# ChainBreak/denoising_diffusion_deep_fake

Hardware: NVIDIA B200
Metric: train_img_per_s (higher is better)
Workload: dtype bf16

## Files before the change

### denoising_diffusion_deep_fake_b200/csrc/common.cuh

```cuda
#pragma once
#include <cuda_runtime.h>
#include <cuda_bf16.h>
#include <stdint.h>
#include <stdio.h>
#include <string.h>
#include "../../include/d3fk.h"

namespace d3fk {

extern int64_t g_launch_count;
extern char g_last_error[512];
extern int* g_dev_error_flag;

int set_error(int code, const char* fmt, ...);
int check_launch(const char* what);
inline void count_launch(int n = 1) { g_launch_count += n; }

#define D3FK_CHECK_ARG(cond, msg)                                        \
  do {                                                                   \
    if (!(cond)) return d3fk::set_error(D3FK_ERR_ARG, "%s: %s", __func__, msg); \
  } while (0)

static inline int cdiv(long long a, long long b) { return (int)((a + b - 1) / b); }

extern int g_use_pdl;
template <typename... KArgs, typename... Args>
static inline cudaError_t launch_k(void (*kernel)(KArgs...), dim3 grid, dim3 block, size_t smem, cudaStream_t s, dim3 cluster,
                                   Args&&... args) {
  cudaLaunchConfig_t cfg;
  memset(&cfg, 0, sizeof(cfg));
  cfg.gridDim = grid;
  cfg.blockDim = block;
  cfg.dynamicSmemBytes = smem;
  cfg.stream = s;
  cudaLaunchAttribute attr[2];
  int na = 0;
  if (cluster.x * cluster.y * cluster.z > 1) {
    attr[na].id = cudaLaunchAttributeClusterDimension;
    attr[na].val.clusterDim.x = cluster.x;
    attr[na].val.clusterDim.y = cluster.y;
    attr[na].val.clusterDim.z = cluster.z;
    ++na;
  }
  if (g_use_pdl) {
    attr[na].id = cudaLaunchAttributeProgrammaticStreamSerialization;
    attr[na].val.programmaticStreamSerializationAllowed = 1;
    ++na;
  }
  cfg.attrs = attr;
  cfg.numAttrs = na;
  return cudaLaunchKernelEx(&cfg, kernel, static_cast<KArgs>(args)...);
}
#ifdef __CUDACC__
__device__ __forceinline__ void grid_barrier_arrive_wait(unsigned* counter, unsigned expected, int* errflag) {
  asm volatile("red.release.gpu.global.add.u32 [%0], 1;" ::"l"(counter) : "memory");
  const long long t0 = clock64();
  while (true) {
    unsigned v;
    asm volatile("ld.acquire.gpu.global.u32 %0, [%1];" : "=r"(v) : "l"(counter) : "memory");
    if (v >= expected) break;
    if (clock64() - t0 > 4000000000ll) {
      atomicExch(errflag, 2);
      printf("[d3fk] grid barrier timeout: block %d of %d saw %u arrivals (expected %u), counter %p\n", (int)blockIdx.x, (int)gridDim.x, v,
             expected, (void*)counter);
      __trap();
    }
  }
}

__device__ __forceinline__ void pdl_enter() {
  asm volatile("griddepcontrol.wait;" ::: "memory");
  asm volatile("griddepcontrol.launch_dependents;" ::: "memory");
}
#endif

template <typename T> struct Vec;
template <> struct Vec<float> {
  static constexpr int N = 4;
  float v[4];
};
template <> struct Vec<__nv_bfloat16> {
  static constexpr int N = 8;
  __nv_bfloat16 v[8];
};

template <typename T> __device__ __forceinline__ float to_f(T x);
template <> __device__ __forceinline__ float to_f<float>(float x) { return x; }
template <> __device__ __forceinline__ float to_f<__nv_bfloat16>(__nv_bfloat16 x) { return __bfloat162float(x); }
template <typename T> __device__ __forceinline__ T from_f(float x);
template <> __device__ __forceinline__ float from_f<float>(float x) { return x; }
template <> __device__ __forceinline__ __nv_bfloat16 from_f<__nv_bfloat16>(float x) { return __float2bfloat16_rn(x); }

template <typename T> __device__ __forceinline__ void load_vec(const T* p, float* out) {
  constexpr int N = Vec<T>::N;
  uint4 raw = *reinterpret_cast<const uint4*>(p);
  const T* e = reinterpret_cast<const T*>(&raw);
#pragma unroll
  for (int i = 0; i < N; ++i) out[i] = to_f<T>(e[i]);
}
template <typename T> __device__ __forceinline__ uint4 load_raw(const T* p) { return *reinterpret_cast<const uint4*>(p); }
template <typename T> __device__ __forceinline__ void unpack_vec(const uint4& raw, float* out) {
  constexpr int N = Vec<T>::N;
  const T* e = reinterpret_cast<const T*>(&raw);
#pragma unroll
  for (int i = 0; i < N; ++i) out[i] = to_f<T>(e[i]);
}
template <typename T> __device__ __forceinline__ void store_vec(T* p, const float* in) {
  constexpr int N = Vec<T>::N;
  uint4 raw;
  T* e = reinterpret_cast<T*>(&raw);
#pragma unroll
  for (int i = 0; i < N; ++i) e[i] = from_f<T>(in[i]);
  *reinterpret_cast<uint4*>(p) = raw;
}

__device__ __forceinline__ uint4 philox4x32_10(uint4 c, uint2 k) {
  const uint32_t M0 = 0xD2511F53u, M1 = 0xCD9E8D57u, W0 = 0x9E3779B9u, W1 = 0xBB67AE85u;
#pragma unroll
  for (int r = 0; r < 10; ++r) {
    uint32_t hi0 = __umulhi(M0, c.x), lo0 = M0 * c.x;
    uint32_t hi1 = __umulhi(M1, c.z), lo1 = M1 * c.z;
    c = make_uint4(hi1 ^ c.y ^ k.x, lo1, hi0 ^ c.w ^ k.y, lo0);
    k.x += W0;
    k.y += W1;
  }
  return c;
}
__device__ __forceinline__ float u32_to_uniform(uint32_t u) { return ((float)u + 0.5f) * 2.3283064365386963e-10f; }
__device__ __forceinline__ float4 philox_normal4(uint64_t seed, uint64_t idx, uint64_t offset) {
  uint4 c = make_uint4((uint32_t)idx, (uint32_t)(idx >> 32), (uint32_t)offset, (uint32_t)(offset >> 32));
  uint4 r = philox4x32_10(c, make_uint2((uint32_t)seed, (uint32_t)(seed >> 32)));
  float u0 = u32_to_uniform(r.x), u1 = u32_to_uniform(r.y), u2 = u32_to_uniform(r.z), u3 = u32_to_uniform(r.w);
  float ra = sqrtf(-2.f * __logf(u0)), rb = sqrtf(-2.f * __logf(u2));
  float s0, c0, s1, c1;
  __sincosf(6.283185307179586f * u1, &s0, &c0);
  __sincosf(6.283185307179586f * u3, &s1, &c1);
  return make_float4(ra * c0, ra * s0, rb * c1, rb * s1);
}

struct Gather {
  const void* src0; const void* src1;
  int c0, c1, ld0, ld1, up0;
  int B, Hi, Wi, Ho, Wo, kh, kw, stride, pad, mode;
  int ctot;
  int K;
  int M;
  int sshift;
};

__device__ __forceinline__ long long gather_offset(const Gather& g, int n, int h0, int w0, int khi, int kwi, int c,
// ... 28 lines not shown
```

### denoising_diffusion_deep_fake_b200/csrc/conv_tc.cu

```cuda
#include "tc_common.cuh"

namespace d3fk {

template <int BN, int PATH, int FUSE> struct ConvCfg {
  static constexpr int STAGES = BN >= 128 ? ((PATH == 2 && FUSE == 3) ? 6 : 3) : 4;
  static constexpr int B_STAGE_BYTES = BN * 128;
  static constexpr int SMEM = 1024 + STAGES * (A_STAGE_BYTES + B_STAGE_BYTES) + 256 + 10 * BN * 4;
  static constexpr int ACC_COLS = BN < 32 ? 32 : BN;
  static constexpr int TMEM_COLS = 2 * ACC_COLS;
};

struct TileSched {
  int MT, NT, KS, kb_per_split, nkb, total, a_ca;
  int bw, bh, bn, wt, ht;
  int off_w, off_h;
  int a_pitch;
};

__device__ __forceinline__ void decode_tile(const TileSched& ts, int t, int& mt, int& nt, int& ks) {
  if (ts.KS > 1) {
    ks = t % ts.KS;
    const int r = t / ts.KS;
    mt = r % ts.MT;
    nt = r / ts.MT;
  } else {
    ks = 0;
    mt = t % ts.MT;
    nt = t / ts.MT;
  }
}

struct FuseBN {
  const float* gamma; const float* beta;
  float* mean; float* invstd; float* running_mean; float* running_var; long long* nbt;
  float* scale; float* shift;
  bf16* act; const bf16* res;
  unsigned* barrier;
  long long count;
  int ldact, ldr, relu;
  float eps, momentum;
};

template <int BN, int PATH, int FUSE>
__global__ void __launch_bounds__(TC_THREADS, 2) conv_tc_kernel(Gather g, FastDiv dWo, FastDiv dHo, const __grid_constant__ CUtensorMap tmA,
                                                             const __grid_constant__ CUtensorMap tmB, EpiTC e, TileSched ts,
                                                             FuseBN fb, int* errflag) {
  using Cfg = ConvCfg<BN, PATH, FUSE>;
  constexpr int STAGES = Cfg::STAGES;
  constexpr int CW = BN >= 32 ? 32 : 16;
  extern __shared__ uint8_t smem_raw[];
  const uint32_t base = (smem_u32(smem_raw) + 1023u) & ~1023u;
  const uint32_t a_base = base;
  const uint32_t b_base = base + STAGES * A_STAGE_BYTES;
  const uint32_t bar_base = b_base + STAGES * Cfg::B_STAGE_BYTES;
  uint8_t* gen_bar = smem_raw + (base - smem_u32(smem_raw)) + STAGES * (A_STAGE_BYTES + Cfg::B_STAGE_BYTES);
  volatile uint32_t* tmem_ptr_slot = reinterpret_cast<volatile uint32_t*>(gen_bar + 8 * (2 * STAGES + 4));
  float* s_stat = reinterpret_cast<float*>(gen_bar + 256);
  float* s_aff = s_stat + 8 * BN;
  constexpr bool affine = FUSE == 3;
  auto full_bar = [&](int s) { return bar_base + 8u * s; };
  auto empty_bar = [&](int s) { return bar_base + 8u * (STAGES + s); };
  auto acc_full_bar = [&](int b) { return bar_base + 8u * (2 * STAGES + b); };
  auto acc_empty_bar = [&](int b) { return bar_base + 8u * (2 * STAGES + 2 + b); };
  const uint32_t recv_bar = bar_base + 8u * (2 * STAGES + 5);

  const int tid = threadIdx.x, warp = warp_index_uniform(), lane = tid & 31;
  const bool is_epi = warp < 4 || warp >= 6;
  const int q = warp & 3;
  const int half = warp >= 6 ? 1 : 0;
  const int etid = warp < 4 ? tid : 128 + (tid - 192);
  auto stage_affine = [&](int nt, bool live) {
    asm volatile("bar.sync 1, 256;" ::: "memory");
    const int ch = nt * BN + etid;
    if (etid < BN) {
      s_aff[etid] = e.scale ? (live && ch < e.Cout ? __ldg(e.scale + ch) : 0.f) : 1.f;
      s_aff[BN + etid] = live && ch < e.Cout ? __ldg(e.shift + ch) : 0.f;
    }
    asm volatile("bar.sync 1, 256;" ::: "memory");
  };
  const bool clus = ts.KS > 1;
  const bool do_stats = e.stats != nullptr;
  TL_DECL
  TL_BEGIN

  if (tid == 0) {
    for (int s = 0; s < STAGES; ++s) {
      mbar_init(full_bar(s), PATH == 2 ? 1 : 129);
      mbar_init(empty_bar(s), 1);
    }
    for (int b = 0; b < 2; ++b) {
      mbar_init(acc_full_bar(b), 1);
      mbar_init(acc_empty_bar(b), EPI_THREADS);
    }
    mbar_init(recv_bar, 1);
    fence_barrier_init();
  }
  if (is_epi) {
    for (int i = etid; i < 8 * BN; i += EPI_THREADS) s_stat[i] = 0.f;
  }
  if (warp == 5 && elect_one_sync()) {
    tma_prefetch_desc(&tmB);
    if (PATH == 2) tma_prefetch_desc(&tmA);
    int mt0, nt0, ks0;
    decode_tile(ts, blockIdx.x, mt0, nt0, ks0);
    const int kbp = ks0 * ts.kb_per_split;
    for (int i = 0; i < STAGES && kbp + i < ts.nkb; ++i) tma_prefetch_l2_2d(&tmB, (kbp + i) * TC_BK, nt0 * BN);
  }
  if (FUSE == 2 && is_epi && e.bw_x) {
    int mt0, nt0, ks0;
    decode_tile(ts, blockIdx.x, mt0, nt0, ks0);
    const long long mp = (long long)mt0 * TC_BM + q * 32 + lane;
    if (mp < g.M) {
      for (int b = half * 128; b < BN * 2; b += 256) {
        prefetch_l2(reinterpret_cast<const char*>(e.bw_x + mp * e.bw_ldx + nt0 * BN) + b);
        if (e.bw_relu) prefetch_l2(reinterpret_cast<const char*>(e.bw_act + mp * e.bw_ldact + nt0 * BN) + b);
      }
    }
  }
  if (warp == 4) tmem_alloc(smem_u32((const void*)tmem_ptr_slot), Cfg::TMEM_COLS);
  tc_fence_before();
  __syncthreads();
  tc_fence_after();
  const uint32_t tmem_d = *tmem_ptr_slot;
  if (tid == 0) { TL_STAMP(1) }

  auto flush_stats = [&](int nt) {
    asm volatile("bar.sync 1, 256;" ::: "memory");
    const int n0 = nt * BN;
    if (tid < BN && n0 + tid < e.Cout) {
      const float a = (s_stat[tid] + s_stat[2 * BN + tid]) + (s_stat[4 * BN + tid] + s_stat[6 * BN + tid]);
      const float b = (s_stat[BN + tid] + s_stat[3 * BN + tid]) + (s_stat[5 * BN + tid] + s_stat[7 * BN + tid]);
      if (a != 0.f || b != 0.f) {
        atomicAdd(&e.stats[n0 + tid], (double)a);
        atomicAdd(&e.stats[e.Cout + n0 + tid], (FUSE == 2 && e.bw_x) ? bw_second_sum((double)a, (double)b, e, n0 + tid) : (double)b);
      }
    }
    asm volatile("bar.sync 1, 256;" ::: "memory");
    for (int i = etid; i < 8 * BN; i += EPI_THREADS) s_stat[i] = 0.f;
    asm volatile("bar.sync 1, 256;" ::: "memory");
  };

  auto fuse_finalize = [&](int nt, bool publisher) {
    asm volatile("bar.sync 1, 256;" ::: "memory");
    if (tid == 0) grid_barrier_arrive_wait(fb.barrier, gridDim.x, errflag);
    asm volatile("bar.sync 1, 256;" ::: "memory");
    const int ch = nt * BN + tid;
    if (tid < BN && ch < e.Cout) {
      const double n = (double)fb.count;
      const double mean = __ldcg(e.stats + ch) / n;
      double var = __ldcg(e.stats + e.Cout + ch) / n - mean * mean;
      if (var < 0) var = 0;
      const double invstd = rsqrt(var + (double)fb.eps);
      const double gm = (double)__ldg(fb.gamma + ch), bt = (double)__ldg(fb.beta + ch);
      s_stat[tid] = (float)(gm * invstd);
      s_stat[BN + tid] = (float)(bt - mean * gm * invstd);
      if (publisher) {
        fb.mean[ch] = (float)mean;
        fb.invstd[ch] = (float)invstd;
        if (fb.scale) { fb.scale[ch] = s_stat[tid]; fb.shift[ch] = s_stat[BN + tid]; }
        if (fb.running_mean) {
          const double unbiased = n > 1 ? var * n / (n - 1) : var;
          fb.running_mean[ch] = (float)((1.0 - fb.momentum) * fb.running_mean[ch] + fb.momentum * mean);
          fb.running_var[ch] = (float)((1.0 - fb.momentum) * fb.running_var[ch] + fb.momentum * unbiased);
        }
        if (ch == 0 && fb.nbt) *fb.nbt += 1;
      }
    }
    asm volatile("bar.sync 1, 256;" ::: "memory");
  };
  auto fuse_apply = [&](float* f, int ncol, long long m, bool row_ok, int nt, int ct) {
    if (!row_ok) return;
    const int cbase = nt * BN + ct;
    for (int q = 0; q < ncol / 8; ++q) {
      float y[8];
#pragma unroll
      for (int i = 0; i < 8; ++i)
        y[i] = fmaf(__bfloat162float(__float2bfloat16_rn(f[q * 8 + i])), s_stat[ct + q * 8 + i], s_stat[BN + ct + q * 8 + i]);
      if (fb.res) {
        const uint4 rr = __ldg(reinterpret_cast<const uint4*>(fb.res + m * fb.ldr + cbase + q * 8));
        const bf16* rb16 = reinterpret_cast<const bf16*>(&rr);
#pragma unroll
        for (int i = 0; i < 8; ++i) y[i] += __bfloat162float(rb16[i]);
      }
      if (fb.relu) {
#pragma unroll
        for (int i = 0; i < 8; ++i) y[i] = fmaxf(y[i], 0.f);
      }
      uint4 o;
      __nv_bfloat162* o2 = reinterpret_cast<__nv_bfloat162*>(&o);
#pragma unroll
      for (int i = 0; i < 4; ++i) o2[i] = __floats2bfloat162_rn(y[2 * i], y[2 * i + 1]);
      *reinterpret_cast<uint4*>(fb.act + m * fb.ldact + cbase + q * 8) = o;
    }
  };

  if (warp == 5) {
    pdl_enter();
    if (tid == 160) { TL_STAMP(2) }
    if (elect_one_sync()) {
      uint32_t kbg = 0;
      const int sgn = g.mode ? -1 : 1;
      for (int t = blockIdx.x; t < ts.total; t += gridDim.x) {
        int mt, nt, ks;
        decode_tile(ts, t, mt, nt, ks);
        const int kb0 = ks * ts.kb_per_split;
        const int kb1 = min(ts.nkb, kb0 + ts.kb_per_split);
        int w0 = 0, h0 = 0, i0 = 0, tap = 0, c = 0, khi = 0, kwi = 0;
        if (PATH == 2) {
          const int tw = mt % ts.wt;
          const int r2 = mt / ts.wt;
          w0 = tw * ts.bw + ts.off_w;
          h0 = (r2 % ts.ht) * ts.bh + ts.off_h;
          i0 = (r2 / ts.ht) * ts.bn;
          const int k = kb0 * TC_BK;
          tap = k / g.ctot;
          c = k - tap * g.ctot;
          khi = tap / g.kw;
          kwi = tap - khi * g.kw;
        }
        for (int kb = kb0; kb < kb1; ++kb, ++kbg) {
          const int s = kbg % STAGES;
          if (kbg >= STAGES) mbar_wait(empty_bar(s), ((kbg / STAGES) - 1) & 1, errflag);
          mbar_arrive_expect_tx(full_bar(s), Cfg::B_STAGE_BYTES + (PATH == 2 ? A_STAGE_BYTES : 0));
          tma_load_2d(b_base + s * Cfg::B_STAGE_BYTES, &tmB, kb * TC_BK, nt * BN, full_bar(s));
          if (PATH == 2) {
            tma_load_4d(a_base + s * A_STAGE_BYTES, &tmA, c, w0 + sgn * kwi, h0 + sgn * khi, i0, full_bar(s));
            c += TC_BK;
            if (c >= g.ctot) {
              c = 0;
              if (++kwi == g.kw) { kwi = 0; ++khi; }
            }
          }
        }
      }
    }
    __syncwarp();
    if (clus) cluster_sync_relaxed();
  } else if (warp == 4) {
    pdl_enter();
    if (elect_one_sync()) {
      constexpr uint32_t idesc = make_idesc(TC_BM, BN, 0, 0);
      uint32_t kbg = 0, tile_iter = 0;
      for (int t = blockIdx.x; t < ts.total; t += gridDim.x, ++tile_iter) {
        int mt, nt, ks;
        decode_tile(ts, t, mt, nt, ks);
        const int kb0 = ks * ts.kb_per_split;
        const int kb1 = min(ts.nkb, kb0 + ts.kb_per_split);
        const uint32_t abuf = tile_iter & 1;
        if (tile_iter >= 2) {
          mbar_wait(acc_empty_bar(abuf), ((tile_iter >> 1) - 1) & 1, errflag);
          tc_fence_after();
        }
        const uint32_t d_addr = tmem_d + abuf * Cfg::ACC_COLS;
        for (int kb = kb0; kb < kb1; ++kb, ++kbg) {
          const int s = kbg % STAGES;
          mbar_wait(full_bar(s), (kbg / STAGES) & 1, errflag);
          if (kbg == 0) { TL_STAMP(3) }
          tc_fence_after();
          const uint32_t a_addr = a_base + s * A_STAGE_BYTES;
          const uint32_t b_addr = b_base + s * Cfg::B_STAGE_BYTES;
#pragma unroll
          for (int kk = 0; kk < TC_BK / 16; ++kk) {
// ... 37 lines not shown
        const int kb1 = min(ts.nkb, kb0 + ts.kb_per_split);

        if (PATH != 2 && warp < 4 && live) {
          int rh[8], rw[8];
          int rn[8];
          const bf16* rp[8];
#pragma unroll
          for (int i = 0; i < 8; ++i) {
            const int m = m0 + rb + 16 * i;
            int n = 0, h0 = -(1 << 28), w0 = 0;
            if (m < g.M) {
              const uint32_t qq = fdiv((uint32_t)m, dWo);
              const int wo = m - (int)qq * g.Wo;
              n = (int)fdiv(qq, dHo);
              const int ho = (int)qq - n * g.Ho;
              if (g.mode == 0) { h0 = ho * g.stride - g.pad; w0 = wo * g.stride - g.pad; }
              else { h0 = ho + g.pad; w0 = wo + g.pad; }
            }
            rh[i] = h0; rw[i] = w0;
            if (PATH == 0) rp[i] = (const bf16*)g.src0 + ((long long)(n * g.Hi + h0) * g.Wi + w0) * g.ld0;
            else rn[i] = n;
          }
          int k = kb0 * TC_BK + j * 8;
          int tap = k / g.ctot;
          int c = k - tap * g.ctot;
          int khi = tap / g.kw, kwi = tap - khi * g.kw;

          for (int kb = kb0; kb < kb1; ++kb, ++kbg) {
            const int s = kbg % STAGES;
            if (kbg >= STAGES) mbar_wait(empty_bar(s), ((kbg / STAGES) - 1) & 1, errflag);
            const bool k_ok = k < g.K;
            const uint32_t a_dst = a_base + s * A_STAGE_BYTES + rb * 128 + sw;
            const int dkh = sgn * khi, dkw = sgn * kwi;
            if (PATH == 0) {
              const long long koff = (long long)(dkh * g.Wi + dkw) * g.ld0 + c;
#pragma unroll
              for (int i = 0; i < 8; ++i) {
                const bool ok = k_ok && (unsigned)(rh[i] + dkh) < (unsigned)g.Hi && (unsigned)(rw[i] + dkw) < (unsigned)g.Wi;
                const void* src = ok ? (const void*)(rp[i] + koff) : g.src0;
                if (ts.a_ca) cp_async_16_ca(a_dst + i * (16 * 128), src, ok ? 16u : 0u);
                else cp_async_16(a_dst + i * (16 * 128), src, ok ? 16u : 0u);
              }
            } else {
              const bool second = c >= g.c0;
              const bf16* sb = second ? (const bf16*)g.src1 + (c - g.c0) : (const bf16*)g.src0 + c;
              const int ld = second ? g.ld1 : g.ld0;
              const int up = second ? 0 : g.up0;
              const int hs = g.Hi >> up, wsz = g.Wi >> up;
#pragma unroll
              for (int i = 0; i < 8; ++i) {
                const int th = rh[i] + dkh, tw = rw[i] + dkw;
                const int hi = th >> sshift, wi = tw >> sshift;
                const bool ok = k_ok && (((uint32_t)(th | tw)) & (0x80000000u | smask)) == 0 && hi < g.Hi && wi < g.Wi;
                const long long pix = (long long)((rn[i] * hs + (hi >> up)) * wsz + (wi >> up));
                const void* src = ok ? (const void*)(sb + pix * ld) : g.src0;
                if (ts.a_ca) cp_async_16_ca(a_dst + i * (16 * 128), src, ok ? 16u : 0u);
                else cp_async_16(a_dst + i * (16 * 128), src, ok ? 16u : 0u);
              }
            }
            cp_async_mbar_arrive(full_bar(s));
            mbar_arrive(full_bar(s));
            k += TC_BK;
            c += TC_BK;
            while (c >= g.ctot) {
              c -= g.ctot;
              if (++kwi == g.kw) { kwi = 0; ++khi; }
            }
          }
        }

        const uint32_t abuf = tile_iter & 1;
        if (live) {
          mbar_wait(acc_full_bar(abuf), (tile_iter >> 1) & 1, errflag);
          if (tid == 0) { TL_STAMP(5) }
          tc_fence_after();
        }
        const int m = m0 + row;
        const bool row_ok = live && m < g.M;
        if (!clus) {
          if (affine && (cur_aff_nt != nt || !live)) {
            stage_affine(nt, live);
            cur_aff_nt = live ? nt : -1;
          }
          if (live && do_stats && cur_nt != nt) {
            if (cur_nt >= 0) flush_stats(cur_nt);
            cur_nt = nt;
          }
          int on = 0, oh = 0, ow = 0;
          if (e.out_nchw && row_ok) {
            const uint32_t qq = fdiv((uint32_t)m, dWo);
            ow = m - (int)qq * e.Wo;
            on = (int)fdiv(qq, dHo);
            oh = (int)qq - on * e.Ho;
          }
#pragma unroll 1
          for (int cc = half * CW; cc < BN; cc += 2 * CW) {
            uint32_t raw[CW];
            const uint32_t taddr = tmem_d + ((uint32_t)(q * 32) << 16) + abuf * Cfg::ACC_COLS + (uint32_t)cc;
            const bool tstats = do_stats && !(FUSE == 2 && e.bw_x);
            if (tstats) tmem_col_stats<CW>(taddr, live ? g.M - (m0 + q * 32) : 0, s_stat + q * 2 * BN + cc, s_stat + q * 2 * BN + BN + cc, lane);
            if (CW == 32) tmem_ld32(taddr, raw); else tmem_ld16(taddr, raw);
            tmem_ld_wait();
            float f[CW];
#pragma unroll
            for (int i = 0; i < CW; ++i) f[i] = __uint_as_float(raw[i]);
            epilogue_chunk<CW, FUSE == 2>(f, e, (long long)m, row_ok, n0 + cc, on, oh, ow, do_stats && !tstats, s_stat + q * 2 * BN + cc,
                                          s_stat + q * 2 * BN + BN + cc, lane, affine ? s_aff + cc : nullptr, BN);
            if (tid == 0 && cc == 0) { TL_STAMP(8) }
          }
          if (tid == 0) { TL_STAMP(9) }
          if (FUSE == 1 && live) {
            flush_stats(nt);
            cur_nt = -1;
            fuse_finalize(nt, mt == 0);
#pragma unroll 1
            for (int cc = half * CW; cc < BN; cc += 2 * CW) {
              uint32_t raw[CW];
              const uint32_t taddr = tmem_d + ((uint32_t)(q * 32) << 16) + abuf * Cfg::ACC_COLS + (uint32_t)cc;
              if (CW == 32) tmem_ld32(taddr, raw); else tmem_ld16(taddr, raw);
              tmem_ld_wait();
              float f[CW];
#pragma unroll
              for (int i = 0; i < CW; ++i) f[i] = __uint_as_float(raw[i]);
              fuse_apply(f, CW, (long long)m, row_ok, nt, cc);
            }
          }
          if (live) {
            tc_fence_before();
            mbar_arrive(acc_empty_bar(abuf));
          }
        } else {
          const int KS = ts.KS, SL = BN / KS, sl4 = SL >> 2;
          const uint32_t rank = cluster_ctarank();
          const uint32_t recv = a_base;
          if (live) {
            if (etid == 0) mbar_arrive_expect_tx(recv_bar, (uint32_t)(TC_BM * BN * 4));
            tc_fence_before();
            cluster_sync_relaxed();
            tc_fence_after();
            if (tid == 0) { TL_STAMP(11) }
          }
#pragma unroll 1
          for (int cc = half * CW; cc < BN; cc += 2 * CW) {
            uint32_t raw[CW];
            const uint32_t taddr = tmem_d + ((uint32_t)(q * 32) << 16) + (uint32_t)cc;
            if (CW == 32) tmem_ld32(taddr, raw); else tmem_ld16(taddr, raw);
            tmem_ld_wait();
#pragma unroll
            for (int q4 = 0; q4 < CW / 4; ++q4) {
              const int col = cc + 4 * q4;
              const int owner = col / SL, within = col - owner * SL;
              const uint32_t la = recv + (uint32_t)((((int)rank * sl4 + (within >> 2)) * 128 + row) * 16);
              const uint32_t ra = mapa_shared(la, (uint32_t)owner);
              if (live) st_async_f4(ra, raw[4 * q4], raw[4 * q4 + 1], raw[4 * q4 + 2], raw[4 * q4 + 3], mapa_shared(recv_bar, (uint32_t)owner));
            }
          }
          if (live) {
            if (tid == 0) { TL_STAMP(12) }
            mbar_wait(recv_bar, 0, errflag);
            if (tid == 0) { TL_STAMP(13) }
          }
          if (affine) stage_affine(nt, live);
          const int cslice = (int)rank * SL;
#pragma unroll 1
          for (int ch = half * 16; ch < SL; ch += 32) {
            float f[16];
#pragma unroll
            for (int c4 = 0; c4 < 4; ++c4) {
              float4 a = make_float4(0.f, 0.f, 0.f, 0.f);
              for (int r = 0; r < KS; ++r) {
                const float4 v = ld_shared_f4(recv + (uint32_t)(((r * sl4 + (ch >> 2) + c4) * 128 + row) * 16));
                a.x += v.x; a.y += v.y; a.z += v.z; a.w += v.w;
              }
              f[4 * c4] = a.x; f[4 * c4 + 1] = a.y; f[4 * c4 + 2] = a.z; f[4 * c4 + 3] = a.w;
            }
            const int ct = cslice + ch;
            const bool tstats = do_stats && !(FUSE == 2 && e.bw_x);
            if (tstats) {
              const uint32_t taddr = tmem_d + ((uint32_t)(q * 32) << 16) + (uint32_t)ct;
              if (live) tmem_st16(taddr, f);
              __syncwarp();
              tmem_col_stats<16>(taddr, live ? g.M - (m0 + q * 32) : 0, s_stat + q * 2 * BN + ct, s_stat + q * 2 * BN + BN + ct, lane);
            }
            epilogue_chunk<16, FUSE == 2>(f, e, (long long)m, row_ok, nt * BN + ct, 0, 0, 0, do_stats && !tstats, s_stat + q * 2 * BN + ct,
                                          s_stat + q * 2 * BN + BN + ct, lane, affine ? s_aff + ct : nullptr, BN);
          }
          if (tid == 0) { TL_STAMP(14) }
          if (live && do_stats) flush_stats(nt);
          if (tid == 0) { TL_STAMP(15) }
          if (FUSE == 1 && live) {
            fuse_finalize(nt, mt == 0 && rank == 0);
#pragma unroll 1
            for (int ch = half * 16; ch < SL; ch += 32) {
              float f[16];
#pragma unroll
              for (int c4 = 0; c4 < 4; ++c4) {
                float4 a = make_float4(0.f, 0.f, 0.f, 0.f);
                for (int r = 0; r < KS; ++r) {
                  const float4 v = ld_shared_f4(recv + (uint32_t)(((r * sl4 + (ch >> 2) + c4) * 128 + row) * 16));
                  a.x += v.x; a.y += v.y; a.z += v.z; a.w += v.w;
                }
                f[4 * c4] = a.x; f[4 * c4 + 1] = a.y; f[4 * c4 + 2] = a.z; f[4 * c4 + 3] = a.w;
              }
              fuse_apply(f, 16, (long long)m, row_ok, nt, cslice + ch);
            }
          }
        }
        if (!live || clus) break;
      }
      if (tid == 0) { TL_STAMP(10) }
      if (live && !clus && do_stats && cur_nt >= 0) flush_stats(cur_nt);
    }
  }

  if (tid == 0) { TL_STAMP(6) }
  tc_fence_before();
  __syncthreads();
  if (warp == 4) tmem_dealloc(tmem_d, Cfg::TMEM_COLS);
  if (tid == 128) { TL_STAMP(7) }
}

int g_num_sms = 148;
int g_verbose = 0;
int g_max_cluster = 8;
static int g_tile_loop = 1;
static int g_a_ca = 0;
static int g_occ_cap = 0;
static int g_use_tma_a = 1;
static int g_split_tiles = 74;
static int g_split_cta_cap = 100;

struct FuseReq { const d3fk_bn_params* bn; unsigned* barrier; bool taken; };
static thread_local FuseReq* t_fuse = nullptr;
static int g_fuse_bn = 1;

template <int BN, int PATH>
static int launch_conv_tc_bn(const Gather& g, const d3fk_conv_params* p, cudaStream_t s, const TileSched& box) {
  EpiTC e{(bf16*)p->out, p->out_nchw, p->scale, p->shift, (const bf16*)p->res, p->stats, p->ldo, p->ldr, p->relu, p->Cout, p->Ho, p->Wo,
           (const bf16*)p->bw_x, (const bf16*)p->bw_act, p->bw_mean, p->bw_invstd, p->bw_ldx, p->bw_ldact, p->bw_relu};
  TileSched ts = box;
  ts.MT = cdiv(g.M, TC_BM);
  ts.NT = cdiv(p->Cout, BN);
  ts.nkb = cdiv(g.K, TC_BK);
  ts.KS = 1;
  const int tiles = ts.MT * ts.NT;
  ts.a_ca = g_a_ca && p->kh > 1;
  if (BN == 128 && !p->out_nchw && p->Cout % BN == 0 && tiles <= g_split_tiles && ts.nkb >= 8 && g_max_cluster > 1) {
    int ks = 1;
    while (ks * 2 <= g_max_cluster && ks * 2 <= 8 && tiles * ks * 2 <= g_split_cta_cap * g_num_sms / 100 && ts.nkb / (ks * 2) >= 4) ks *= 2;
    while (ks > 1 && tiles * ks > cluster_capacity(ks, 2)) ks >>= 1;
    ts.KS = ks;
  }
  ts.kb_per_split = cdiv(ts.nkb, ts.KS);
  if (ts.KS > 1 && (ts.KS - 1) * ts.kb_per_split >= ts.nkb) {
    ts.KS = 1;
    ts.kb_per_split = ts.nkb;
  }
  ts.total = tiles * ts.KS;
  const bool eval_affine = !p->bw_x && (p->scale || p->shift);
  const int smem_bytes = eval_affine ? ConvCfg<BN, PATH, 3>::SMEM : ConvCfg<BN, PATH, 0>::SMEM;
  int occ = (227 * 1024) / (smem_bytes + 1024);
  if (occ * ConvCfg<BN, PATH, 0>::TMEM_COLS > 512) occ = 512 / ConvCfg<BN, PATH, 0>::TMEM_COLS;
  if (g_occ_cap > 0 && occ > g_occ_cap) occ = g_occ_cap;
  int grid = ts.total < g_num_sms * occ ? ts.total : g_num_sms * occ;
  if (!g_tile_loop || ts.KS > 1) grid = ts.total;

  alignas(64) CUtensorMap tmA, tmB;
  memset(&tmA, 0, sizeof(tmA));
  {
    uint64_t dims[2] = {(uint64_t)g.K, (uint64_t)p->Cout};
    uint64_t strides[1] = {(uint64_t)g.K * 2};
    uint32_t bx[2] = {TC_BK, (uint32_t)BN};
    int rc = get_tensor_map(&tmB, p->w, 2, dims, strides, bx, 128);
    if (rc) return rc;
  }
  if (PATH == 2) {
    uint64_t dims[4] = {(uint64_t)g.c0, (uint64_t)g.Wi, (uint64_t)g.Hi, (uint64_t)g.B};
    const uint64_t pitch = (uint64_t)(ts.a_pitch ? ts.a_pitch : g.Wi);
    uint64_t strides[3] = {(uint64_t)g.ld0 * 2, pitch * g.ld0 * 2, (uint64_t)g.Hi * pitch * g.ld0 * 2};
    uint32_t bx[4] = {TC_BK, (uint32_t)ts.bw, (uint32_t)ts.bh, (uint32_t)ts.bn};
    int rc = get_tensor_map(&tmA, p->src0, 4, dims, strides, bx, 128);
    if (rc) return rc;
  }
  FuseBN fb;
  memset(&fb, 0, sizeof(fb));
  bool fuse = false;
  if (BN == 128 && t_fuse && g_fuse_bn && p->stats && !p->scale && !p->shift && !p->res && !p->relu && !p->out_nchw && p->mode == 0 &&
      p->Cout % BN == 0 && ts.total <= cluster_capacity_safe(ts.KS)) {
// ... 183 lines not shown
```

### denoising_diffusion_deep_fake_b200/csrc/tc_common.cuh

```cuda
#pragma once
#include <stdlib.h>
#include <string.h>
#include "common.cuh"
#include "tma.cuh"

namespace d3fk {

typedef __nv_bfloat16 bf16;

#ifdef D3FK_TIMELINE
#define TL_SLOTS 16
#define TL_MAX 512
__device__ __forceinline__ unsigned long long tl_now() { unsigned long long t; asm volatile("mov.u64 %0, %%globaltimer;" : "=l"(t)); return t; }
#define TL_DECL unsigned long long* tl_buf = reinterpret_cast<unsigned long long*>(errflag + 16); __shared__ unsigned tl_idx;
#define TL_BEGIN if (blockIdx.x == 0 && threadIdx.x == 0) { tl_idx = atomicAdd(reinterpret_cast<unsigned*>(errflag + 4), 1u) % TL_MAX; tl_buf[tl_idx * TL_SLOTS + 0] = tl_now(); }
#define TL_STAMP(slot) if (blockIdx.x == 0) { tl_buf[tl_idx * TL_SLOTS + (slot)] = tl_now(); }
#else
#define TL_DECL
#define TL_BEGIN
#define TL_STAMP(slot)
#endif

__device__ __forceinline__ uint32_t smem_u32(const void* p) { return (uint32_t)__cvta_generic_to_shared(p); }

__device__ __forceinline__ bool elect_one_sync() {
  uint32_t pred;
  asm volatile("{\n\t.reg .pred p;\n\telect.sync _|p, 0xffffffff;\n\tselp.u32 %0, 1, 0, p;\n\t}" : "=r"(pred));
  return pred != 0;
}
__device__ __forceinline__ int warp_index_uniform() { return __shfl_sync(0xffffffffu, (int)(threadIdx.x >> 5), 0); }

__device__ __forceinline__ void mbar_init(uint32_t bar, uint32_t count) {
  asm volatile("mbarrier.init.shared::cta.b64 [%0], %1;" ::"r"(bar), "r"(count) : "memory");
}
__device__ __forceinline__ void mbar_arrive(uint32_t bar) {
  asm volatile("mbarrier.arrive.shared::cta.b64 _, [%0];" ::"r"(bar) : "memory");
}
__device__ __forceinline__ void cp_async_mbar_arrive(uint32_t bar) {
  asm volatile("cp.async.mbarrier.arrive.shared::cta.b64 [%0];" ::"r"(bar) : "memory");
}
__device__ __forceinline__ uint32_t mbar_try_wait(uint32_t bar, uint32_t parity) {
  uint32_t ok;
  asm volatile(
      "{\n\t.reg .pred p;\n\t"
      "mbarrier.try_wait.parity.shared::cta.b64 p, [%1], %2;\n\t"
      "selp.u32 %0, 1, 0, p;\n\t}"
      : "=r"(ok)
      : "r"(bar), "r"(parity)
      : "memory");
  return ok;
}
static __device__ __noinline__ void mbar_timeout(int* errflag, uint32_t bar, uint32_t parity) {
  atomicExch(errflag, 1);
  printf("[d3fk] mbarrier watchdog: block %d thread %d waited > 2 s on barrier 0x%x parity %u\n", (int)blockIdx.x,
         (int)threadIdx.x, bar, parity);
  __trap();
}
__device__ __forceinline__ void mbar_wait(uint32_t bar, uint32_t parity, int* errflag) {
  if (mbar_try_wait(bar, parity)) return;
  unsigned long long t0;
  asm volatile("mov.u64 %0, %%globaltimer;" : "=l"(t0));
  for (uint32_t it = 1;; ++it) {
    if (mbar_try_wait(bar, parity)) return;
    if ((it & 1023u) == 0) {
      unsigned long long t;
      asm volatile("mov.u64 %0, %%globaltimer;" : "=l"(t));
      if (t - t0 > 2000000000ull) mbar_timeout(errflag, bar, parity);
    }
  }
}
__device__ __forceinline__ void cp_async_16(uint32_t dst, const void* src, uint32_t bytes) {
  asm volatile("cp.async.cg.shared.global [%0], [%1], 16, %2;" ::"r"(dst), "l"(src), "r"(bytes) : "memory");
}
__device__ __forceinline__ void cp_async_16_ca(uint32_t dst, const void* src, uint32_t bytes) {
  asm volatile("cp.async.ca.shared.global [%0], [%1], 16, %2;" ::"r"(dst), "l"(src), "r"(bytes) : "memory");
}
__device__ __forceinline__ void fence_proxy_async() { asm volatile("fence.proxy.async.shared::cta;" ::: "memory"); }
__device__ __forceinline__ void fence_barrier_init() { asm volatile("fence.mbarrier_init.release.cluster;" ::: "memory"); }
__device__ __forceinline__ void tc_fence_before() { asm volatile("tcgen05.fence::before_thread_sync;" ::: "memory"); }
__device__ __forceinline__ void tc_fence_after() { asm volatile("tcgen05.fence::after_thread_sync;" ::: "memory"); }

__device__ __forceinline__ void tmem_alloc(uint32_t smem_dst, uint32_t ncols) {
  asm volatile("tcgen05.alloc.cta_group::1.sync.aligned.shared::cta.b32 [%0], %1;" ::"r"(smem_dst), "r"(ncols) : "memory");
  asm volatile("tcgen05.relinquish_alloc_permit.cta_group::1.sync.aligned;" ::: "memory");
}
__device__ __forceinline__ void tmem_dealloc(uint32_t taddr, uint32_t ncols) {
  asm volatile("tcgen05.dealloc.cta_group::1.sync.aligned.b32 %0, %1;" ::"r"(taddr), "r"(ncols) : "memory");
}
__device__ __forceinline__ void umma_f16(uint32_t d_tmem, uint64_t adesc, uint64_t bdesc, uint32_t idesc, uint32_t accumulate) {
  asm volatile(
      "{\n\t.reg .pred p;\n\t"
      "setp.ne.b32 p, %4, 0;\n\t"
      "tcgen05.mma.cta_group::1.kind::f16 [%0], %1, %2, %3, p;\n\t}"
      ::"r"(d_tmem), "l"(adesc), "l"(bdesc), "r"(idesc), "r"(accumulate)
      : "memory");
}
__device__ __forceinline__ void umma_f16_lohi(uint32_t d_tmem, uint32_t alo, uint32_t ahi, uint32_t blo, uint32_t bhi, uint32_t idesc,
                                              uint32_t accumulate) {
  asm volatile(
      "{\n\t.reg .pred p;\n\t.reg .b64 da, db;\n\t"
      "mov.b64 da, {%1, %2};\n\t"
      "mov.b64 db, {%3, %4};\n\t"
      "setp.ne.b32 p, %6, 0;\n\t"
      "tcgen05.mma.cta_group::1.kind::f16 [%0], da, db, %5, p;\n\t}"
      ::"r"(d_tmem), "r"(alo), "r"(ahi), "r"(blo), "r"(bhi), "r"(idesc), "r"(accumulate)
      : "memory");
}
__device__ __forceinline__ void umma_commit(uint32_t bar) {
  asm volatile("tcgen05.commit.cta_group::1.mbarrier::arrive::one.shared::cluster.b64 [%0];" ::"r"(bar) : "memory");
}
__device__ __forceinline__ void tmem_ld32(uint32_t taddr, uint32_t* v) {
  asm volatile(
      "tcgen05.ld.sync.aligned.32x32b.x32.b32 "
      "{%0, %1, %2, %3, %4, %5, %6, %7, %8, %9, %10, %11, %12, %13, %14, %15, "
      "%16, %17, %18, %19, %20, %21, %22, %23, %24, %25, %26, %27, %28, %29, %30, %31}, [%32];"
      : "=r"(v[0]), "=r"(v[1]), "=r"(v[2]), "=r"(v[3]), "=r"(v[4]), "=r"(v[5]), "=r"(v[6]), "=r"(v[7]), "=r"(v[8]),
        "=r"(v[9]), "=r"(v[10]), "=r"(v[11]), "=r"(v[12]), "=r"(v[13]), "=r"(v[14]), "=r"(v[15]), "=r"(v[16]),
        "=r"(v[17]), "=r"(v[18]), "=r"(v[19]), "=r"(v[20]), "=r"(v[21]), "=r"(v[22]), "=r"(v[23]), "=r"(v[24]),
        "=r"(v[25]), "=r"(v[26]), "=r"(v[27]), "=r"(v[28]), "=r"(v[29]), "=r"(v[30]), "=r"(v[31])
      : "r"(taddr)
      : "memory");
}
__device__ __forceinline__ void tmem_ld16(uint32_t taddr, uint32_t* v) {
  asm volatile(
      "tcgen05.ld.sync.aligned.32x32b.x16.b32 "
      "{%0, %1, %2, %3, %4, %5, %6, %7, %8, %9, %10, %11, %12, %13, %14, %15}, [%16];"
      : "=r"(v[0]), "=r"(v[1]), "=r"(v[2]), "=r"(v[3]), "=r"(v[4]), "=r"(v[5]), "=r"(v[6]), "=r"(v[7]), "=r"(v[8]),
        "=r"(v[9]), "=r"(v[10]), "=r"(v[11]), "=r"(v[12]), "=r"(v[13]), "=r"(v[14]), "=r"(v[15])
      : "r"(taddr)
      : "memory");
}
__device__ __forceinline__ void tmem_ld_wait() { asm volatile("tcgen05.wait::ld.sync.aligned;" ::: "memory"); }

__device__ __forceinline__ uint32_t cluster_ctarank() {
  uint32_t r;
  asm volatile("mov.u32 %0, %%cluster_ctarank;" : "=r"(r));
  return r;
}
__device__ __forceinline__ void cluster_sync_all() {
  asm volatile("barrier.cluster.arrive.release.aligned;\n\tbarrier.cluster.wait.acquire.aligned;" ::: "memory");
}
__device__ __forceinline__ void cluster_sync_relaxed() {
  asm volatile("barrier.cluster.arrive.relaxed.aligned;\n\tbarrier.cluster.wait.aligned;" ::: "memory");
}
__device__ __forceinline__ void st_async_f4(uint32_t remote_addr, uint32_t a, uint32_t b, uint32_t c, uint32_t d, uint32_t remote_mbar) {
  asm volatile("st.async.weak.shared::cluster.mbarrier::complete_tx::bytes.v4.b32 [%0], {%1, %2, %3, %4}, [%5];"
               ::"r"(remote_addr), "r"(a), "r"(b), "r"(c), "r"(d), "r"(remote_mbar) : "memory");
}
__device__ __forceinline__ uint32_t mapa_shared(uint32_t addr, uint32_t rank) {
  uint32_t r;
  asm volatile("mapa.shared::cluster.u32 %0, %1, %2;" : "=r"(r) : "r"(addr), "r"(rank));
  return r;
}
__device__ __forceinline__ void st_cluster_f4(uint32_t addr, uint32_t a, uint32_t b, uint32_t c, uint32_t d) {
  asm volatile("st.shared::cluster.v4.b32 [%0], {%1, %2, %3, %4};" ::"r"(addr), "r"(a), "r"(b), "r"(c), "r"(d) : "memory");
}
__device__ __forceinline__ float4 ld_shared_f4(uint32_t addr) {
  float4 v;
  asm volatile("ld.shared.v4.f32 {%0, %1, %2, %3}, [%4];" : "=f"(v.x), "=f"(v.y), "=f"(v.z), "=f"(v.w) : "r"(addr) : "memory");
  return v;
}

__device__ __forceinline__ uint64_t make_smem_desc(uint32_t saddr, uint32_t lbo_bytes, uint32_t sbo_bytes) {
  uint64_t d = 0;
  d |= (uint64_t)((saddr & 0x3FFFFu) >> 4);
  d |= (uint64_t)((lbo_bytes >> 4) & 0x3FFFu) << 16;
  d |= (uint64_t)((sbo_bytes >> 4) & 0x3FFFu) << 32;
  d |= (uint64_t)1 << 46;
  d |= (uint64_t)2 << 61;
  return d;
}
__host__ __device__ constexpr uint32_t make_idesc(int M, int N, int a_mn_major, int b_mn_major) {
  return (1u << 4) | (1u << 7) | (1u << 10) | ((uint32_t)a_mn_major << 15) | ((uint32_t)b_mn_major << 16) |
         ((uint32_t)(N >> 3) << 17) | ((uint32_t)(M >> 4) << 24);
}

__device__ __forceinline__ float warp_colsum32(float* v, int lane) {
#pragma unroll
  for (int ofs = 16, n = 32; ofs >= 1; ofs >>= 1, n >>= 1) {
    const bool up = (lane & ofs) != 0;
#pragma unroll
    for (int i = 0; i < n / 2; ++i) {
      float send = up ? v[i] : v[i + n / 2];
      float keep = up ? v[i + n / 2] : v[i];
      v[i] = keep + __shfl_xor_sync(0xffffffffu, send, ofs);
    }
  }
  return v[0];
}
__device__ __forceinline__ float warp_colsum16(float* v, int lane) {
#pragma unroll
  for (int i = 0; i < 16; ++i) v[i] += __shfl_xor_sync(0xffffffffu, v[i], 16);
#pragma unroll
  for (int ofs = 8, n = 16; ofs >= 1; ofs >>= 1, n >>= 1) {
    const bool up = (lane & ofs) != 0;
#pragma unroll
    for (int i = 0; i < n / 2; ++i) {
      float send = up ? v[i] : v[i + n / 2];
      float keep = up ? v[i + n / 2] : v[i];
      v[i] = keep + __shfl_xor_sync(0xffffffffu, send, ofs);
    }
  }
  return v[0];
}

template <int NREP> __device__ __forceinline__ void tmem_ld_16x256b(uint32_t taddr, uint32_t* v);
template <> __device__ __forceinline__ void tmem_ld_16x256b<4>(uint32_t taddr, uint32_t* v) {
  asm volatile(
      "tcgen05.ld.sync.aligned.16x256b.x4.b32 "
      "{%0, %1, %2, %3, %4, %5, %6, %7, %8, %9, %10, %11, %12, %13, %14, %15}, [%16];"
      : "=r"(v[0]), "=r"(v[1]), "=r"(v[2]), "=r"(v[3]), "=r"(v[4]), "=r"(v[5]), "=r"(v[6]), "=r"(v[7]), "=r"(v[8]),
        "=r"(v[9]), "=r"(v[10]), "=r"(v[11]), "=r"(v[12]), "=r"(v[13]), "=r"(v[14]), "=r"(v[15])
      : "r"(taddr)
      : "memory");
}
template <> __device__ __forceinline__ void tmem_ld_16x256b<2>(uint32_t taddr, uint32_t* v) {
  asm volatile("tcgen05.ld.sync.aligned.16x256b.x2.b32 {%0, %1, %2, %3, %4, %5, %6, %7}, [%8];"
               : "=r"(v[0]), "=r"(v[1]), "=r"(v[2]), "=r"(v[3]), "=r"(v[4]), "=r"(v[5]), "=r"(v[6]), "=r"(v[7])
               : "r"(taddr)
               : "memory");
}
__device__ __forceinline__ void tmem_st16(uint32_t taddr, const float* f) {
  asm volatile(
      "tcgen05.st.sync.aligned.32x32b.x16.b32 [%0], {%1, %2, %3, %4, %5, %6, %7, %8, %9, %10, %11, %12, %13, %14, %15, %16};"
      ::"r"(taddr), "f"(f[0]), "f"(f[1]), "f"(f[2]), "f"(f[3]), "f"(f[4]), "f"(f[5]), "f"(f[6]), "f"(f[7]), "f"(f[8]), "f"(f[9]),
        "f"(f[10]), "f"(f[11]), "f"(f[12]), "f"(f[13]), "f"(f[14]), "f"(f[15])
      : "memory");
  asm volatile("tcgen05.wait::st.sync.aligned;" ::: "memory");
}
template <int CW>
__device__ __forceinline__ void tmem_col_stats(uint32_t taddr, int row_limit, float* sstat_sum, float* sstat_sq, int lane) {
  constexpr int J = CW / 8;
  uint32_t a[4 * J], b[4 * J];
  tmem_ld_16x256b<J>(taddr, a);
  tmem_ld_16x256b<J>(taddr + (16u << 16), b);
  tmem_ld_wait();
  const int r0 = lane >> 2;
  const bool v0 = r0 < row_limit, v1 = r0 + 8 < row_limit, v2 = r0 + 16 < row_limit, v3 = r0 + 24 < row_limit;
// ... 183 lines not shown
```

Measured before the change: 73970.

## Split fused-BN grid barrier into arrive/wait and overlap with epilogue work

The fused conv+BN epilogue (FUSE==1) previously did a combined arrive-and-wait grid barrier before any output processing. The barrier is now split: each block arrives right after accumulating its channel stats. While other blocks arrive, it prefetches residual tiles into shared memory via cp.async, loads gamma/beta and running stats, and runs a pre-barrier output pass. It then waits and applies normalization with the staged residual and vectorized scale/shift reads. This hides barrier latency and global residual-load latency, at the cost of a second TMEM read pass and reuse of A-stage shared memory as residual staging. The cluster split-K path also seems to drop its old cross-rank reduction sum in favor of reading TMEM directly.

```diff
diff --git a/denoising_diffusion_deep_fake_b200/csrc/common.cuh b/denoising_diffusion_deep_fake_b200/csrc/common.cuh
--- a/denoising_diffusion_deep_fake_b200/csrc/common.cuh
+++ b/denoising_diffusion_deep_fake_b200/csrc/common.cuh
@@ -52,8 +52,10 @@
   return cudaLaunchKernelEx(&cfg, kernel, static_cast<KArgs>(args)...);
 }
 #ifdef __CUDACC__
-__device__ __forceinline__ void grid_barrier_arrive_wait(unsigned* counter, unsigned expected, int* errflag) {
+__device__ __forceinline__ void grid_barrier_arrive(unsigned* counter) {
   asm volatile("red.release.gpu.global.add.u32 [%0], 1;" ::"l"(counter) : "memory");
+}
+__device__ __forceinline__ void grid_barrier_wait(unsigned* counter, unsigned expected, int* errflag) {
   const long long t0 = clock64();
   while (true) {
     unsigned v;
@@ -66,6 +68,10 @@
       __trap();
     }
   }
+}
+__device__ __forceinline__ void grid_barrier_arrive_wait(unsigned* counter, unsigned expected, int* errflag) {
+  grid_barrier_arrive(counter);
+  grid_barrier_wait(counter, expected, errflag);
 }
 
 __device__ __forceinline__ void pdl_enter() {
diff --git a/denoising_diffusion_deep_fake_b200/csrc/conv_tc.cu b/denoising_diffusion_deep_fake_b200/csrc/conv_tc.cu
--- a/denoising_diffusion_deep_fake_b200/csrc/conv_tc.cu
+++ b/denoising_diffusion_deep_fake_b200/csrc/conv_tc.cu
@@ -47,6 +47,8 @@
                                                              FuseBN fb, int* errflag) {
   using Cfg = ConvCfg<BN, PATH, FUSE>;
   constexpr int STAGES = Cfg::STAGES;
+  static_assert(FUSE != 1 || (STAGES * A_STAGE_BYTES >= TC_BM * BN * 2 &&
+                              STAGES * (A_STAGE_BYTES + Cfg::B_STAGE_BYTES) >= TC_BM * BN * 5), "FUSE 1 residual staging");
   constexpr int CW = BN >= 32 ? 32 : 16;
   extern __shared__ uint8_t smem_raw[];
   const uint32_t base = (smem_u32(smem_raw) + 1023u) & ~1023u;
@@ -67,6 +69,7 @@
   const int tid = threadIdx.x, warp = warp_index_uniform(), lane = tid & 31;
   const bool is_epi = warp < 4 || warp >= 6;
   const int q = warp & 3;
+  const int erow = q * 32 + lane;
   const int half = warp >= 6 ? 1 : 0;
   const int etid = warp < 4 ? tid : 128 + (tid - 192);
   auto stage_affine = [&](int nt, bool live) {
@@ -140,44 +143,85 @@
     asm volatile("bar.sync 1, 256;" ::: "memory");
   };
 
-  auto fuse_finalize = [&](int nt, bool publisher) {
+  auto fuse_arrive = [&](int nt, bool live) {
     asm volatile("bar.sync 1, 256;" ::: "memory");
-    if (tid == 0) grid_barrier_arrive_wait(fb.barrier, gridDim.x, errflag);
+    const int n0 = nt * BN;
+    if (live && tid < BN && n0 + tid < e.Cout) {
+      const float a = (s_stat[tid] + s_stat[2 * BN + tid]) + (s_stat[4 * BN + tid] + s_stat[6 * BN + tid]);
+      const float b = (s_stat[BN + tid] + s_stat[3 * BN + tid]) + (s_stat[5 * BN + tid] + s_stat[7 * BN + tid]);
+      if (a != 0.f || b != 0.f) {
+        atomicAdd(&e.stats[n0 + tid], (double)a);
+        atomicAdd(&e.stats[e.Cout + n0 + tid], (double)b);
+      }
+    }
     asm volatile("bar.sync 1, 256;" ::: "memory");
-    const int ch = nt * BN + tid;
-    if (tid < BN && ch < e.Cout) {
+    if (tid == 0) { TL_STAMP(16) }
+    if (live && tid == 0) grid_barrier_arrive(fb.barrier);
+    if (tid == 0) { TL_STAMP(17) }
+  };
+  const int fch = tid;
+  float f_gamma = 0.f, f_beta = 0.f, f_rmean = 0.f, f_rvar = 0.f;
+  double f_mean = 0.0, f_var = 0.0, f_invstd = 0.0;
+  auto fuse_load_params = [&](int nt, bool publisher) {
+    const int ch = nt * BN + fch;
+    if (fch < BN && ch < e.Cout) {
+      f_gamma = __ldg(fb.gamma + ch);
+      f_beta = __ldg(fb.beta + ch);
+      if (publisher && fb.running_mean) { f_rmean = fb.running_mean[ch]; f_rvar = fb.running_var[ch]; }
+    }
+  };
+  auto fuse_wait = [&](int nt) {
+    if (tid == 0) grid_barrier_wait(fb.barrier, gridDim.x, errflag);
+    if (tid == 0) { TL_STAMP(18) }
+    asm volatile("bar.sync 1, 256;" ::: "memory");
+    const int ch = nt * BN + fch;
+    if (fch < BN && ch < e.Cout) {
       const double n = (double)fb.count;
-      const double mean = __ldcg(e.stats + ch) / n;
-      double var = __ldcg(e.stats + e.Cout + ch) / n - mean * mean;
-      if (var < 0) var = 0;
-      const double invstd = rsqrt(var + (double)fb.eps);
-      const double gm = (double)__ldg(fb.gamma + ch), bt = (double)__ldg(fb.beta + ch);
-      s_stat[tid] = (float)(gm * invstd);
-      s_stat[BN + tid] = (float)(bt - mean * gm * invstd);
-      if (publisher) {
-        fb.mean[ch] = (float)mean;
-        fb.invstd[ch] = (float)invstd;
-        if (fb.scale) { fb.scale[ch] = s_stat[tid]; fb.shift[ch] = s_stat[BN + tid]; }
-        if (fb.running_mean) {
-          const double unbiased = n > 1 ? var * n / (n - 1) : var;
-          fb.running_mean[ch] = (float)((1.0 - fb.momentum) * fb.running_mean[ch] + fb.momentum * mean);
-          fb.running_var[ch] = (float)((1.0 - fb.momentum) * fb.running_var[ch] + fb.momentum * unbiased);
-        }
-        if (ch == 0 && fb.nbt) *fb.nbt += 1;
-      }
+      f_mean = __ldcg(e.stats + ch) / n;
+      f_var = __ldcg(e.stats + e.Cout + ch) / n - f_mean * f_mean;
+      if (f_var < 0) f_var = 0;
+      f_invstd = rsqrt(f_var + (double)fb.eps);
+      const double gm = (double)f_gamma, bt = (double)f_beta;
+      s_stat[fch] = (float)(gm * f_invstd);
+      s_stat[BN + fch] = (float)(bt - f_mean * gm * f_invstd);
     }
     asm volatile("bar.sync 1, 256;" ::: "memory");
+    if (tid == 0) { TL_STAMP(19) }
   };
-  auto fuse_apply = [&](float* f, int ncol, long long m, bool row_ok, int nt, int ct) {
+  auto fuse_publish = [&](int nt) {
+    const int ch = nt * BN + fch;
+    if (fch < BN && ch < e.Cout) {
+      fb.mean[ch] = (float)f_mean;
+      fb.invstd[ch] = (float)f_invstd;
+      if (fb.scale) { fb.scale[ch] = s_stat[fch]; fb.shift[ch] = s_stat[BN + fch]; }
+      if (fb.running_mean) {
+        const double n = (double)fb.count;
+        const double unbiased = n > 1 ? f_var * n / (n - 1) : f_var;
+        fb.running_mean[ch] = (float)((1.0 - fb.momentum) * f_rmean + fb.momentum * f_mean);
+        fb.running_var[ch] = (float)((1.0 - fb.momentum) * f_rvar + fb.momentum * unbiased);
+      }
+      if (ch == 0 && fb.nbt) *fb.nbt += 1;
+    }
+  };
+  auto fuse_fetch_res = [&](uint32_t res_s, long long m, bool row_ok, int cbase, int cj, int ncol) {
+    if (!fb.res || !row_ok) return;
+    for (int q8 = 0; q8 < ncol / 8; ++q8)
+      cp_async_16(res_s + (uint32_t)(((cj + q8) * TC_BM + erow) * 16), fb.res + m * fb.ldr + cbase + q8 * 8, 16u);
+  };
+  auto fuse_apply = [&](float* f, int ncol, long long m, bool row_ok, int nt, int ct, uint32_t res_s, int cj) {
     if (!row_ok) return;
     const int cbase = nt * BN + ct;
     for (int q = 0; q < ncol / 8; ++q) {
-      float y[8];
+      float y[8], sc[8], sh[8];
+      *reinterpret_cast<float4*>(sc) = *reinterpret_cast<const float4*>(s_stat + ct + q * 8);
+      *reinterpret_cast<float4*>(sc + 4) = *reinterpret_cast<const float4*>(s_stat + ct + q * 8 + 4);
+      *reinterpret_cast<float4*>(sh) = *reinterpret_cast<const float4*>(s_stat + BN + ct + q * 8);
+      *reinterpret_cast<float4*>(sh + 4) = *reinterpret_cast<const float4*>(s_stat + BN + ct + q * 8 + 4);
 #pragma unroll
       for (int i = 0; i < 8; ++i)
-        y[i] = fmaf(__bfloat162float(__float2bfloat16_rn(f[q * 8 + i])), s_stat[ct + q * 8 + i], s_stat[BN + ct + q * 8 + i]);
+        y[i] = fmaf(__bfloat162float(__float2bfloat16_rn(f[q * 8 + i])), sc[i], sh[i]);
       if (fb.res) {
-        const uint4 rr = __ldg(reinterpret_cast<const uint4*>(fb.res + m * fb.ldr + cbase + q * 8));
+        const uint4 rr = ld_shared_u4(res_s + (uint32_t)(((cj + q) * TC_BM + erow) * 16));
         const bf16* rb16 = reinterpret_cast<const bf16*>(&rr);
 #pragma unroll
         for (int i = 0; i < 8; ++i) y[i] += __bfloat162float(rb16[i]);
@@ -381,7 +425,7 @@
             stage_affine(nt, live);
             cur_aff_nt = live ? nt : -1;
           }
-          if (live && do_stats && cur_nt != nt) {
+          if (FUSE != 1 && live && do_stats && cur_nt != nt) {
             if (cur_nt >= 0) flush_stats(cur_nt);
             cur_nt = nt;
           }
@@ -392,37 +436,58 @@
             on = (int)fdiv(qq, dHo);
             oh = (int)qq - on * e.Ho;
           }
+          if (FUSE == 1) {
+            const uint32_t tbase = tmem_d + ((uint32_t)(q * 32) << 16) + abuf * Cfg::ACC_COLS;
 #pragma unroll 1
-          for (int cc = half * CW; cc < BN; cc += 2 * CW) {
-            uint32_t raw[CW];
-            const uint32_t taddr = tmem_d + ((uint32_t)(q * 32) << 16) + abuf * Cfg::ACC_COLS + (uint32_t)cc;
-            const bool tstats = do_stats && !(FUSE == 2 && e.bw_x);
-            if (tstats) tmem_col_stats<CW>(taddr, live ? g.M - (m0 + q * 32) : 0, s_stat + q * 2 * BN + cc, s_stat + q * 2 * BN + BN + cc, lane);
-            if (CW == 32) tmem_ld32(taddr, raw); else tmem_ld16(taddr, raw);
-            tmem_ld_wait();
-            float f[CW];
-#pragma unroll
-            for (int i = 0; i < CW; ++i) f[i] = __uint_as_float(raw[i]);
-            epilogue_chunk<CW, FUSE == 2>(f, e, (long long)m, row_ok, n0 + cc, on, oh, ow, do_stats && !tstats, s_stat + q * 2 * BN + cc,
-                                          s_stat + q * 2 * BN + BN + cc, lane, affine ? s_aff + cc : nullptr, BN);
-            if (tid == 0 && cc == 0) { TL_STAMP(8) }
-          }
-          if (tid == 0) { TL_STAMP(9) }
-          if (FUSE == 1 && live) {
-            flush_stats(nt);
-            cur_nt = -1;
-            fuse_finalize(nt, mt == 0);
+            for (int cc = half * CW; cc < BN; cc += 2 * CW)
+              tmem_col_stats<CW>(tbase + (uint32_t)cc, live ? g.M - (m0 + q * 32) : 0,
+                                 s_stat + q * 2 * BN + cc, s_stat + q * 2 * BN + BN + cc, lane);
+            if (tid == 0) { TL_STAMP(9) }
+            fuse_arrive(nt, live);
+            if (live) fuse_load_params(nt, mt == 0);
+#pragma unroll 1
+            for (int cc = half * CW; cc < BN; cc += 2 * CW) {
+              fuse_fetch_res(a_base, (long long)m, row_ok, n0 + cc, cc / 8, CW);
+              uint32_t raw[CW];
+              if (CW == 32) tmem_ld32(tbase + (uint32_t)cc, raw); else tmem_ld16(tbase + (uint32_t)cc, raw);
+              tmem_ld_wait();
+              float f[CW];
+#pragma unroll
+              for (int i = 0; i < CW; ++i) f[i] = __uint_as_float(raw[i]);
+              epilogue_chunk<CW, false>(f, e, (long long)m, row_ok, n0 + cc, 0, 0, 0, false, nullptr, nullptr, lane);
+            }
+            if (tid == 0) { TL_STAMP(20) }
+            if (live) fuse_wait(nt);
+            cp_async_wait_all();
+#pragma unroll 1
+            for (int cc = half * CW; cc < BN; cc += 2 * CW) {
+              uint32_t raw[CW];
+              if (CW == 32) tmem_ld32(tbase + (uint32_t)cc, raw); else tmem_ld16(tbase + (uint32_t)cc, raw);
+              tmem_ld_wait();
+              float f[CW];
+#pragma unroll
+              for (int i = 0; i < CW; ++i) f[i] = __uint_as_float(raw[i]);
+              fuse_apply(f, CW, (long long)m, row_ok, nt, cc, a_base, cc / 8);
+            }
+            if (tid == 0) { TL_STAMP(21) }
+            if (live && mt == 0) fuse_publish(nt);
+          } else {
 #pragma unroll 1
             for (int cc = half * CW; cc < BN; cc += 2 * CW) {
               uint32_t raw[CW];
               const uint32_t taddr = tmem_d + ((uint32_t)(q * 32) << 16) + abuf * Cfg::ACC_COLS + (uint32_t)cc;
+              const bool tstats = do_stats && !(FUSE == 2 && e.bw_x);
+              if (tstats) tmem_col_stats<CW>(taddr, live ? g.M - (m0 + q * 32) : 0, s_stat + q * 2 * BN + cc, s_stat + q * 2 * BN + BN + cc, lane);
               if (CW == 32) tmem_ld32(taddr, raw); else tmem_ld16(taddr, raw);
               tmem_ld_wait();
               float f[CW];
 #pragma unroll
               for (int i = 0; i < CW; ++i) f[i] = __uint_as_float(raw[i]);
-              fuse_apply(f, CW, (long long)m, row_ok, nt, cc);
-            }
+              epilogue_chunk<CW, FUSE == 2>(f, e, (long long)m, row_ok, n0 + cc, on, oh, ow, do_stats && !tstats, s_stat + q * 2 * BN + cc,
+                                            s_stat + q * 2 * BN + BN + cc, lane, affine ? s_aff + cc : nullptr, BN);
+              if (tid == 0 && cc == 0) { TL_STAMP(8) }
+            }
+            if (tid == 0) { TL_STAMP(9) }
           }
           if (live) {
             tc_fence_before();
@@ -481,28 +546,48 @@
               __syncwarp();
               tmem_col_stats<16>(taddr, live ? g.M - (m0 + q * 32) : 0, s_stat + q * 2 * BN + ct, s_stat + q * 2 * BN + BN + ct, lane);
             }
-            epilogue_chunk<16, FUSE == 2>(f, e, (long long)m, row_ok, nt * BN + ct, 0, 0, 0, do_stats && !tstats, s_stat + q * 2 * BN + ct,
-                                          s_stat + q * 2 * BN + BN + ct, lane, affine ? s_aff + ct : nullptr, BN);
+            if (FUSE != 1)
+              epilogue_chunk<16, FUSE == 2>(f, e, (long long)m, row_ok, nt * BN + ct, 0, 0, 0, do_stats && !tstats, s_stat + q * 2 * BN + ct,
+                                            s_stat + q * 2 * BN + BN + ct, lane, affine ? s_aff + ct : nullptr, BN);
           }
           if (tid == 0) { TL_STAMP(14) }
-          if (live && do_stats) flush_stats(nt);
-          if (tid == 0) { TL_STAMP(15) }
-          if (FUSE == 1 && live) {
-            fuse_finalize(nt, mt == 0 && rank == 0);
+          if (FUSE == 1) {
+            const bool publisher = mt == 0 && rank == 0;
+            const uint32_t tbase = tmem_d + ((uint32_t)(q * 32) << 16);
+            const uint32_t res_s = a_base + TC_BM * BN * 4;
+            fuse_arrive(nt, live);
+            if (live) fuse_load_params(nt, publisher);
 #pragma unroll 1
             for (int ch = half * 16; ch < SL; ch += 32) {
+              const int ct = cslice + ch;
+              fuse_fetch_res(res_s, (long long)m, row_ok, nt * BN + ct, ch / 8, 16);
+              uint32_t raw[16];
+              tmem_ld16(tbase + (uint32_t)ct, raw);
+              tmem_ld_wait();
               float f[16];
 #pragma unroll
-              for (int c4 = 0; c4 < 4; ++c4) {
-                float4 a = make_float4(0.f, 0.f, 0.f, 0.f);
-                for (int r = 0; r < KS; ++r) {
-                  const float4 v = ld_shared_f4(recv + (uint32_t)(((r * sl4 + (ch >> 2) + c4) * 128 + row) * 16));
-                  a.x += v.x; a.y += v.y; a.z += v.z; a.w += v.w;
-                }
-                f[4 * c4] = a.x; f[4 * c4 + 1] = a.y; f[4 * c4 + 2] = a.z; f[4 * c4 + 3] = a.w;
-              }
-              fuse_apply(f, 16, (long long)m, row_ok, nt, cslice + ch);
-            }
+              for (int i = 0; i < 16; ++i) f[i] = __uint_as_float(raw[i]);
+              epilogue_chunk<16, false>(f, e, (long long)m, row_ok, nt * BN + ct, 0, 0, 0, false, nullptr, nullptr, lane);
+            }
+            if (tid == 0) { TL_STAMP(20) }
+            if (live) fuse_wait(nt);
+            cp_async_wait_all();
+#pragma unroll 1
+            for (int ch = half * 16; ch < SL; ch += 32) {
+              const int ct = cslice + ch;
+              uint32_t raw[16];
+              tmem_ld16(tbase + (uint32_t)ct, raw);
+              tmem_ld_wait();
+              float f[16];
+#pragma unroll
+              for (int i = 0; i < 16; ++i) f[i] = __uint_as_float(raw[i]);
+              fuse_apply(f, 16, (long long)m, row_ok, nt, ct, res_s, ch / 8);
+            }
+            if (tid == 0) { TL_STAMP(21) }
+            if (live && publisher) fuse_publish(nt);
+          } else {
+            if (live && do_stats) flush_stats(nt);
+            if (tid == 0) { TL_STAMP(15) }
           }
         }
         if (!live || clus) break;
diff --git a/denoising_diffusion_deep_fake_b200/csrc/tc_common.cuh b/denoising_diffusion_deep_fake_b200/csrc/tc_common.cuh
--- a/denoising_diffusion_deep_fake_b200/csrc/tc_common.cuh
+++ b/denoising_diffusion_deep_fake_b200/csrc/tc_common.cuh
@@ -9,8 +9,8 @@
 typedef __nv_bfloat16 bf16;
 
 #ifdef D3FK_TIMELINE
-#define TL_SLOTS 16
-#define TL_MAX 512
+#define TL_SLOTS 32
+#define TL_MAX 256
 __device__ __forceinline__ unsigned long long tl_now() { unsigned long long t; asm volatile("mov.u64 %0, %%globaltimer;" : "=l"(t)); return t; }
 #define TL_DECL unsigned long long* tl_buf = reinterpret_cast<unsigned long long*>(errflag + 16); __shared__ unsigned tl_idx;
 #define TL_BEGIN if (blockIdx.x == 0 && threadIdx.x == 0) { tl_idx = atomicAdd(reinterpret_cast<unsigned*>(errflag + 4), 1u) % TL_MAX; tl_buf[tl_idx * TL_SLOTS + 0] = tl_now(); }
@@ -75,6 +75,7 @@
 __device__ __forceinline__ void cp_async_16_ca(uint32_t dst, const void* src, uint32_t bytes) {
   asm volatile("cp.async.ca.shared.global [%0], [%1], 16, %2;" ::"r"(dst), "l"(src), "r"(bytes) : "memory");
 }
+__device__ __forceinline__ void cp_async_wait_all() { asm volatile("cp.async.wait_all;" ::: "memory"); }
 __device__ __forceinline__ void fence_proxy_async() { asm volatile("fence.proxy.async.shared::cta;" ::: "memory"); }
 __device__ __forceinline__ void fence_barrier_init() { asm volatile("fence.mbarrier_init.release.cluster;" ::: "memory"); }
 __device__ __forceinline__ void tc_fence_before() { asm volatile("tcgen05.fence::before_thread_sync;" ::: "memory"); }
@@ -154,6 +155,11 @@
 }
 __device__ __forceinline__ void st_cluster_f4(uint32_t addr, uint32_t a, uint32_t b, uint32_t c, uint32_t d) {
   asm volatile("st.shared::cluster.v4.b32 [%0], {%1, %2, %3, %4};" ::"r"(addr), "r"(a), "r"(b), "r"(c), "r"(d) : "memory");
+}
+__device__ __forceinline__ uint4 ld_shared_u4(uint32_t addr) {
+  uint4 v;
+  asm volatile("ld.shared.v4.b32 {%0, %1, %2, %3}, [%4];" : "=r"(v.x), "=r"(v.y), "=r"(v.z), "=r"(v.w) : "r"(addr) : "memory");
+  return v;
 }
 __device__ __forceinline__ float4 ld_shared_f4(uint32_t addr) {
   float4 v;
```

Result: faster. 75840, median of 6 (+2.5%).
